# pain7576/ddpg-trucktrailer

Hardware: AMD Instinct MI355X
Metric: env-steps/s (higher is better)
Workload: dtype f64

## Files before the change

### ddpg-trucktrailer_amd/_lib.py

```python
import ctypes as C
import os

HERE = os.path.dirname(os.path.abspath(__file__))
LIB_PATH = os.environ.get("TT_LIB_PATH") or os.path.join(HERE, "libttenv.so")

OBS_DIM = 23
MAX_EPISODE_STEPS = 4095
TT_OK, TT_EINVAL, TT_ENOMEM, TT_EHIP, TT_ENODEV = 0, -1, -2, -3, -4
F_JACKKNIFE, F_OUT_OF_MAP, F_MAX_STEPS, F_GOAL_REACHED, F_GOAL_PASSED, F_EXCESSIVE_BACK, F_SUCCESS = (1 << i for i in range(7))
VIOLATIONS = ("none", "jackknife", "jackknife_warning", "major_boundary", "minor_boundary", "past_the_goal",
              "max_step", "excessive_backward")
INFO_ROWS = ("total_reward", "progress_reward", "heading_reward", "orientation_reward", "staged_success",
             "safety_penalty", "exploration_bonus", "final_success_bonus", "backward_penalty", "smoothness_penalty",
             "cumulative_backward", "movement_budget")
NINFO = len(INFO_ROWS)
LOG_COUNTS = ("episodes", "successes", "jackknife", "out_of_map", "max_steps", "goal_reached", "goal_passed",
              "excessive_back", "success_flag")
LOG_DETAIL = 1
LOG_COMPONENTS = INFO_ROWS[1:10]


class TTParams(C.Structure):
    _fields_ = [(n, C.c_double) for n in ("L1", "L2", "hitch_offset", "v1x", "dt", "map_min_x", "map_max_x", "map_min_y",
                                          "map_max_y", "max_steer", "position_threshold", "orientation_threshold",
                                          "step_length")] + \
               [("extra_steps", C.c_int32), ("fixed_max_steps", C.c_int32), ("term_mask", C.c_uint32),
                ("variant", C.c_int32), ("stateless_reward", C.c_int32), ("reserved_", C.c_int32),
                ("goal", C.c_double * 3), ("reset_lo", C.c_double * 3),
                ("reset_hi", C.c_double * 3)]


class TTInfo(C.Structure):
    _fields_ = [("comp", C.c_void_p), ("violation", C.c_void_p), ("flags", C.c_void_p)]


class TTMlpWeights(C.Structure):
    _fields_ = [(n, C.c_void_p) for n in ("w1", "b1", "g1", "be1", "w2", "b2", "g2", "be2", "w3", "b3", "wa", "ba")] + \
               [("in_dim", C.c_int32), ("fc1_dims", C.c_int32), ("fc2_dims", C.c_int32), ("capped_grids", C.c_int32),
                ("split_ws", C.c_void_p), ("ws_packed", C.c_int32), ("max_workgroups", C.c_int32), ("split_ws_alt", C.c_void_p), ("fc2_img", C.c_void_p)]


class TTFc2Images(C.Structure):
    _fields_ = [("net", C.c_void_p), ("target", C.c_void_p)]


class TTMlpSaved(C.Structure):
    _fields_ = [(n, C.c_void_p) for n in ("xh1", "h1", "xh2", "h2", "rstd1", "rstd2")]


class TTFwdJob(C.Structure):
    _fields_ = [("critic", C.c_int32), ("reserved_", C.c_int32), ("obs", C.c_void_p), ("action", C.c_void_p),
                ("w", C.POINTER(TTMlpWeights)), ("out", C.c_void_p), ("saved", C.POINTER(TTMlpSaved)),
                ("dq_da", C.c_void_p), ("z_state", C.c_void_p)]

# ... 145 lines not shown
    "tt_adam_soft_update": (C.c_int, [_I, _P, _P, _P, _P, _P, _P, _P, C.c_float, C.c_float, C.c_float, C.c_float,
                                      C.c_float, C.c_float, C.POINTER(TTFc2Images), _P, _P]),
    "tt_p2p_create": (C.c_int, [_I, _I, _I, _I, _P, C.POINTER(_P)]),
    "tt_p2p_destroy": (C.c_int, [_P]),
    "tt_p2p_export": (C.c_int, [_P, _P]),
    "tt_p2p_attach": (C.c_int, [_P, _I, _P]),
    "tt_p2p_grad": (_P, [_P, _I]),
    "tt_p2p_reset": (C.c_int, [_P, _P]),
    "tt_p2p_set_timeout": (C.c_int, [_P, C.c_double]),
    "tt_p2p_gave_up": (C.c_int, [_P]),
    "tt_p2p_last_error": (C.c_char_p, [_P]),
    "tt_adam_soft_update_p2p": (C.c_int, [_P, _I, _I, _P, _P, _P, _P, _P, _P, C.c_float, C.c_float, C.c_float, C.c_float,
                                          C.c_float, C.c_float, C.POINTER(TTFc2Images), _P, _P]),
    "tt_mlp_fc2_image_bytes": (C.c_uint64, []),
    "tt_mlp_fc2_image_pack": (C.c_int, [C.POINTER(TTMlpWeights), _P]),
    "tt_random_actions": (C.c_int, [_I, _U64, _U64, _P, _P]),
    "tt_pop_learn_create": (C.c_int, [_I, _I, C.POINTER(TTPopAgent), C.POINTER(_P)]),
    "tt_pop_learn": (C.c_int, [_P, _I, _P]),
    "tt_pop_learn_destroy": (C.c_int, [_P]),
    "tt_pop_exploit": (C.c_int, [_P, _I, C.POINTER(TTPopExploitPair), _P]),
    "tt_pop_hyper": (C.c_int, [_P, _I, C.POINTER(C.c_float * 4)]),
    "tt_pop_learn_set_nstep": (C.c_int, [_P, C.POINTER(TTPopNstep)]),
    "tt_pop_exploit_nstep": (C.c_int, [_P, _I, C.POINTER(TTPopExploitPair), C.POINTER(TTPopNstep), _P]),
    "tt_pop_nstep": (C.c_int, [_P, _I, C.POINTER(TTPopNstep)]),
    "tt_learn_log_create": (C.c_int, [_I, _I, C.POINTER(TTLearnLogJob), C.c_int64, C.c_int32, C.POINTER(_P)]),
    "tt_learn_log_append": (C.c_int, [_P, _P]),
    "tt_learn_log_drain": (C.c_int, [_P, _I, C.c_int64, C.c_int64, _P, _P, _P, C.POINTER(C.c_int64)]),
    "tt_learn_log_clear": (C.c_int, [_P, _P]),
    "tt_learn_log_destroy": (C.c_int, [_P]),
    "tt_td3_create": (C.c_int, [_I, C.POINTER(TTTd3Agent), C.POINTER(_P)]),
# ... 53 lines not shown
```

### ddpg-trucktrailer_amd/csrc/ttlearn.hip

```cpp
#include "ttlearn_bodies.h"
#include "ttp2p.h"

namespace {

template <bool CRITIC>
__global__ __launch_bounds__(64 * NW) void k_fwd_small(const int n, const float *__restrict__ obs,
                                                   const float *__restrict__ action, const float *__restrict__ w1e,
                                                   const float *__restrict__ b1e, const float *__restrict__ g1e,
                                                   const float *__restrict__ be1e, const Weights W,
                                                   float *__restrict__ out, const Saved sv, float *__restrict__ dq_da,
                                                   float *__restrict__ z_state) {
    __shared__ __attribute__((aligned(16))) float h1_s[H1S_FLOATS];
    __shared__ __attribute__((aligned(16))) float z_s[TR * DS];
    __shared__ __attribute__((aligned(16))) float w1_s[H1 * IN];
    KernargWarm<64 + (int)sizeof(Weights) + 8 + (int)sizeof(Saved) + 16> warm;
    warm.issue();
    KBEGIN(3);
    const EarlyW E{w1e, b1e, g1e, be1e};
    auto hook = [&]() __attribute__((always_inline)) { warm.wait(); };
    fwd_small_body<CRITIC, decltype(hook)>(n, obs, action, W, out, sv, dq_da, z_state, h1_s, z_s, w1_s, blockIdx.x * TR, nullptr, false, 0.f,
                                           0.f, nullptr, 0u, &E, hook);
    KEND(3);
}

__global__ __launch_bounds__(64 * NW) void k_fwd_multi(const FwdJobs J) {
    __shared__ __attribute__((aligned(16))) float h1_s[H1S_FLOATS];
    __shared__ __attribute__((aligned(16))) float z_s[TR * DS];
    __shared__ __attribute__((aligned(16))) float w1_s[H1 * IN];
    kernarg_warm<(int)sizeof(FwdJobs)>();
    const int job = blockIdx.x / J.blocks_per_job, row0 = (blockIdx.x - job * J.blocks_per_job) * TR;
    const FwdJob &q = J.j[job];
    KBEGIN(0);
#ifdef TT_STAMPS
    if (blockIdx.x == 0 && threadIdx.x < 64) {
        unsigned long long m = 0;
        for (int i = threadIdx.x; i < 512; i += 64) m = max(m, g_kblk[4][i][1]);
        for (int o = 32; o > 0; o >>= 1) m = max(m, (unsigned long long)__shfl_xor((long long)m, o));
        if (threadIdx.x == 0) g_kblk[5][0][0] = m;
    }
// ... 26 lines not shown
                        J.R.a_out[b] = ttnet::ring_pick_a(J.R, p);
                        if (J.R.idx_out) { J.R.idx_out[2 * b] = p.side ? -1 : p.t; J.R.idx_out[2 * b + 1] = p.side ? p.j : p.e; }
                    }
                }
                if (job == J.write_s2) {
                    J.R.s2_out[(size_t)b * ttnet::IN + c] = ttnet::ring_pick_s2(J.R, p)[c];
                    if (c == 0) { J.R.r_out[b] = ttnet::ring_pick_r(J.R, p); J.R.d_out[b] = ttnet::ring_pick_d(J.R, p); }
                }
            }
        }
    }
    if (q.critic)
        fwd_small_body<true>(J.n, q.obs, q.action, q.W, q.out, q.sv, q.dq_da, q.z_state, h1_s, z_s, w1_s, row0, orow, have_act, act_r0, act_r1);
    else
        fwd_small_body<false>(J.n, q.obs, q.action, q.W, q.out, q.sv, nullptr, nullptr, h1_s, z_s, w1_s, row0, orow);
    KEND(0);
}

__global__ __launch_bounds__(64 * NW) void k_bwd_rows_pair(const int n, const float scale_c, const float *__restrict__ q_out,
                                                           const Weights Wc, const Saved sv_c, const BwdOut o_c, const TdIn td,
                                                           const float *__restrict__ mu_out, const Weights Wa, const Saved sv_a,
                                                           const BwdOut o_a, const ImageJob img) {
    __shared__ __attribute__((aligned(16))) float dx2_s[DXS_FLOATS];
    __shared__ float red[2 * NW * TR];
    __shared__ float rsc_s[TR];
    kernarg_warm<16 + 2 * ((int)sizeof(Weights) + (int)sizeof(Saved) + (int)sizeof(BwdOut)) + (int)sizeof(TdIn) + 8>();
    const int nb = (n + TR - 1) / TR;
    if ((int)blockIdx.x == 2 * nb) {
        if (threadIdx.x == 0) clock_tick(td);
        return;
// ... 194 lines not shown
    const int nn = i / H1, k = i - nn * H1;
    img_store(img, nn, k, w2[i], true);
}

}

extern "C" {

int tt_mlp_forward_save(int n, int critic, const float *obs, const float *action, const tt_mlp_weights *w, float *out,
                        const tt_mlp_saved *saved, float *dq_da, tt_stream_t stream) {
    if (n < 0 || !obs || !out || !ok_shape(w, critic != 0) || (critic && !action)) return TT_EINVAL;
    if (n == 0) return TT_OK;
    Saved sv{nullptr, nullptr, nullptr, nullptr, nullptr, nullptr};
    if (saved && !to_saved(saved, sv)) return TT_EINVAL;
    const dim3 grid((n + TR - 1) / TR), block(64 * NW);
    if (critic)
        hipLaunchKernelGGL(k_fwd_small<true>, grid, block, 0, stream, n, obs, action, w->w1, w->b1, w->g1, w->be1, to_weights(w), out, sv, dq_da,
                           static_cast<float *>(nullptr));
    else
        hipLaunchKernelGGL(k_fwd_small<false>, grid, block, 0, stream, n, obs, action, w->w1, w->b1, w->g1, w->be1, to_weights(w), out, sv,
                           static_cast<float *>(nullptr), static_cast<float *>(nullptr));
    return hipGetLastError() == hipSuccess ? TT_OK : TT_EHIP;
}

static int forward_multi_impl(int n, int count, const tt_fwd_job *jobs, const tt_sample_args *sample, int64_t *k_snapshot,
                              tt_stream_t stream) {
    if (n < 0 || count < 1 || count > 4 || !jobs) return TT_EINVAL;
    if (n == 0) return TT_OK;
    FwdJobs J{};
    J.n = n;
    J.blocks_per_job = (n + TR - 1) / TR;
    J.write_s = J.write_s2 = -1;
    if (sample) {
        if (sample->batch != n) return TT_EINVAL;
        const int rc = ttnet::make_ring_sample(sample, J.R);
        if (rc != TT_OK) return rc;
        J.sampled = 1;
        J.R.progress = const_cast<int *>(sample->step_progress);
        J.k_snapshot = reinterpret_cast<long long *>(k_snapshot);
    }
    for (int i = 0; i < count; ++i)
        if (!to_fwd_job(jobs[i], i, sample, J)) return TT_EINVAL;
    if (sample && (J.write_s < 0 || J.write_s2 < 0)) return TT_EINVAL;
    hipLaunchKernelGGL(k_fwd_multi, dim3(count * J.blocks_per_job), dim3(64 * NW), 0, stream, J);
    return hipGetLastError() == hipSuccess ? TT_OK : TT_EHIP;
}

int tt_mlp_forward_multi(int n, int count, const tt_fwd_job *jobs, tt_stream_t stream) {
    return forward_multi_impl(n, count, jobs, nullptr, nullptr, stream);
}

int tt_mlp_forward_multi_sampled(int n, int count, const tt_fwd_job *jobs, const tt_sample_args *sample, int64_t *k_snapshot,
                                 tt_stream_t stream) {
    if (!sample) return TT_EINVAL;
    return forward_multi_impl(n, count, jobs, sample, k_snapshot, stream);
}

int tt_mlp_backward_rows_pair(int n, float scale_critic, const float *q_out, const tt_mlp_weights *critic,
                              const tt_mlp_saved *saved_critic, const tt_mlp_bwd_ws *ws_critic, const tt_td_input *tdi,
// ... 125 lines not shown
    X.world = x->world; X.me = x->rank; X.site = site;
    for (int r = 0; r < x->world; ++r) {
        if (!x->attached[r] || !x->block[r] || !x->flags[r]) return TT_EINVAL;
        X.arrive[r] = reinterpret_cast<int *>(x->flags[r]);
        X.grad[r] = reinterpret_cast<const float *>(x->block[r] + x->offset[site]);
    }
    X.gave_up_host = x->gave_up_host;
    X.wait_ticks = x->wait_ticks;
    hipLaunchKernelGGL(k_adam_soft_p2p, dim3(blocks), dim3(256), 0, stream, T, X, reinterpret_cast<const long long *>(step_dev), lr,
                       beta1, beta2, eps, weight_decay, tau, bias_corr);
    return hipGetLastError() == hipSuccess ? TT_OK : TT_EHIP;
}

uint64_t tt_mlp_fc2_image_bytes(void) { return (uint64_t)IMG_HALVES * 2; }

int tt_mlp_fc2_image_pack(const tt_mlp_weights *w, tt_stream_t stream) {
    if (!w || !w->w2 || !w->fc2_img || w->fc1_dims != H1 || w->fc2_dims != H2) return TT_EINVAL;
    hipLaunchKernelGGL(k_img_pack, dim3((H2 * H1 + 255) / 256), dim3(256), 0, stream, w->w2,
                       reinterpret_cast<_Float16 *>(w->fc2_img));
    return hipGetLastError() == hipSuccess ? TT_OK : TT_EHIP;
}

#ifdef TT_STAMPS
int tt_debug_blocks(unsigned long long *out1024) {
    return hipMemcpyFromSymbol(out1024, HIP_SYMBOL(g_blk), sizeof(unsigned long long) * 1024) == hipSuccess ? 0 : -3;
}
int tt_debug_wst(unsigned long long *out32) {
    return hipMemcpyFromSymbol(out32, HIP_SYMBOL(g_wst), sizeof(unsigned long long) * 32) == hipSuccess ? 0 : -3;
}
int tt_debug_kblocks(unsigned long long *out6x1024) {
// ... 21 lines not shown
```

### ddpg-trucktrailer_amd/csrc/ttlearn_bodies.h

```cpp
#pragma once
#include <hip/hip_runtime.h>

#include <cstdint>

#include "ttenv.h"
#include "ttnet_common.h"
#include "ttnet_pack.h"
#include "ttstamps.h"

namespace {

constexpr int IN = 23, INP = 24;
constexpr int H1 = 400, H2 = 300, H2P = 320, H2K = 304;
constexpr int NT1 = H1 / 16, NT2 = H2P / 16;
constexpr int TR = 16;
constexpr int NW = 8;
constexpr int HS1 = 404;

constexpr int DS = 308;

using f32x4 = __attribute__((ext_vector_type(4))) float;
using f16x8 = __attribute__((ext_vector_type(8))) _Float16;

constexpr int K2P = 416;
// ... 164 lines not shown
__device__ __forceinline__ float4 f4_ldu(const float *p) { return *reinterpret_cast<const float4 *>(p); }
__device__ __forceinline__ float f4_sum(const float4 v) { return (v.x + v.y) + (v.z + v.w); }
using h2v = __attribute__((ext_vector_type(2))) _Float16;
__device__ __forceinline__ void split4(const float4 x, uint2 &ph, uint2 &pm) {
    h2v a, b, c, d;
    a[0] = (_Float16)x.x; a[1] = (_Float16)x.y; b[0] = (_Float16)x.z; b[1] = (_Float16)x.w;
    c[0] = (_Float16)(x.x - (float)a[0]); c[1] = (_Float16)(x.y - (float)a[1]);
    d[0] = (_Float16)(x.z - (float)b[0]); d[1] = (_Float16)(x.w - (float)b[1]);
    ph = make_uint2(__builtin_bit_cast(uint32_t, a), __builtin_bit_cast(uint32_t, b));
    pm = make_uint2(__builtin_bit_cast(uint32_t, c), __builtin_bit_cast(uint32_t, d));
}

struct EarlyW {
    const float *__restrict__ w1, *__restrict__ b1, *__restrict__ g1, *__restrict__ be1;
};
template <bool CRITIC, class Hook = NoHook>
__device__ __forceinline__ void fwd_small_body(const int n, const float *__restrict__ obs,
                                               const float *__restrict__ action, const Weights &W,
                                               float *__restrict__ out, const Saved &sv, float *__restrict__ dq_da,
                                               float *__restrict__ z_state, float *__restrict__ h1_s,
                                               float *__restrict__ z_s, float *__restrict__ w1_s, const int row0,
                                               const float *__restrict__ obs_row_lane = nullptr,
                                               const bool act_given = false, const float act_row0 = 0.f,
                                               const float act_row1 = 0.f, unsigned long long *dq_words = nullptr,
                                               const unsigned dq_epoch = 0u, const EarlyW *early = nullptr,
                                               const Hook &loads_issued = Hook()) {
    const EarlyW E = early ? *early : EarlyW{W.w1, W.b1, W.g1, W.be1};
    const int tid = threadIdx.x, wave = tid >> 6, lane = tid & 63, l15 = lane & 15, l4 = lane >> 4;

    STAMP(0);
    constexpr int MT1 = (NT1 + NW - 1) / NW, MT2 = (NT2 + NW - 1) / NW;
    float4 pb1[RV], pg1[RV], pbe1[RV], pb2[RV], pg2[RV], pbe2[RV], pw3[RV], pwa[RV], pba[RV];
#pragma unroll
    for (int i = 0; i < RV; ++i) {
        const int c = rv_col(lane, i), cc = c < H1 ? c : 0;
        pb1[i] = *reinterpret_cast<const float4 *>(E.b1 + cc); pg1[i] = *reinterpret_cast<const float4 *>(E.g1 + cc);
        pbe1[i] = *reinterpret_cast<const float4 *>(E.be1 + cc);
    }
    f32x4 acc1[MT1];
#pragma unroll
    for (int i = 0; i < MT1; ++i) acc1[i] = f32x4{0.f, 0.f, 0.f, 0.f};
    constexpr int GU_F = 3;
    const bool img = W.img != nullptr;
    const int nt_f = (NT2 - wave + NW - 1) / NW;
    f16x8 bpre[GU_F][MT2][2];
    {
        float a[INP / 4];
        const float *arow = obs_row_lane ? obs_row_lane : obs + (size_t)min(row0 + l15, n - 1) * IN;
        const bool arow_ok = row0 + l15 < n;
        constexpr int W1_F4 = H1 * IN / 4, W1_PER = (W1_F4 + 64 * NW - 1) / (64 * NW);
        float4 wv[W1_PER];
#pragma unroll
        for (int q = 0; q < W1_PER; ++q) wv[q] = f4_ldu(E.w1 + 4 * min(tid + 64 * NW * q, W1_F4 - 1));
#pragma unroll
        for (int ks = 0; ks < INP / 4; ++ks) a[ks] = arow[min(ks * 4 + l4, IN - 1)];
        loads_issued();
        SUB(0);
#pragma unroll
        for (int q = 0; q < W1_PER; ++q)
            if (tid + 64 * NW * q < W1_F4) *reinterpret_cast<float4 *>(w1_s + 4 * (tid + 64 * NW * q)) = wv[q];
// ... 5 lines not shown
        float b[MT1][INP / 4];
#pragma unroll
        for (int i = 0; i < MT1; ++i) {
            const float *wr = w1_s + (min(wave + NW * i, NT1 - 1) * 16 + l15) * IN;
#pragma unroll
            for (int ks = 0; ks < INP / 4; ++ks) {
                const float v = wr[min(ks * 4 + l4, IN - 1)];
                b[i][ks] = ks * 4 + l4 < IN ? v : 0.f;
            }
        }
#pragma unroll
        for (int ks = 0; ks < INP / 4; ++ks)
#pragma unroll
            for (int i = 0; i < MT1; ++i)
                if (wave + NW * i < NT1) acc1[i] = __builtin_amdgcn_mfma_f32_16x16x4f32(a[ks], b[i][ks], acc1[i], 0, 0, 0);
        if (img) {
#pragma unroll
            for (int u = 0; u < GU_F; ++u)
#pragma unroll
                for (int i = 0; i < MT2; ++i) {
                    const _Float16 *bq = W.img + ((size_t)min(wave + NW * i, NT2 - 1) * FW_STEPS * 64 + lane) * 8 + 512 * u;
                    bpre[u][i][0] = *reinterpret_cast<const f16x8 *>(bq);
                    bpre[u][i][1] = *reinterpret_cast<const f16x8 *>(bq + IMG_FWD);
                }
        }
    }
    STAMP(1);
#pragma unroll
    for (int i = 0; i < MT1; ++i) {
        const int t = wave + NW * i;
        if (t < NT1) {
#pragma unroll
            for (int r = 0; r < 4; ++r) h1_s[(l4 * 4 + r) * HS1 + t * 16 + l15] = acc1[i][r];
        }
    }
    SUB(3);
    lds_barrier();
    SUB(4);
    _Float16 *const ap_s = reinterpret_cast<_Float16 *>(h1_s);
// ... 14 lines not shown
#pragma unroll
    for (int rr = 0; rr < TR / NW; ++rr) {
        const int lr = wave * (TR / NW) + rr, row = row0 + lr;
        const float mean = wave_sum64(f4_sum(xr[rr][0]) + f4_sum(xr[rr][1])) * (1.f / H1);
        float4 dv[RV];
        float ss = 0.f;
#pragma unroll
        for (int i = 0; i < RV; ++i) {
            const bool ok = rv_col(lane, i) < H1;
            const float4 x = xr[rr][i];
            dv[i] = ok ? make_float4(x.x - mean, x.y - mean, x.z - mean, x.w - mean) : f4_zero();
            ss = fmaf(dv[i].x, dv[i].x, ss); ss = fmaf(dv[i].y, dv[i].y, ss);
            ss = fmaf(dv[i].z, dv[i].z, ss); ss = fmaf(dv[i].w, dv[i].w, ss);
        }
        const float rstd = rsqrtf(wave_sum64(ss) * (1.f / H1) + 1e-5f);
        if (sv.rstd1 && lane == 0 && row < n) sv.rstd1[row] = rstd;
        const bool save = sv.xh1 && row < n;
#pragma unroll
        for (int i = 0; i < RV; ++i) {
            const int c = rv_col(lane, i);
            if (c < H1) {
                const float4 xh = make_float4(dv[i].x * rstd, dv[i].y * rstd, dv[i].z * rstd, dv[i].w * rstd);
                const float4 h = make_float4(fmaxf(fmaf(xh.x, pg1[i].x, pbe1[i].x), 0.f), fmaxf(fmaf(xh.y, pg1[i].y, pbe1[i].y), 0.f),
                                             fmaxf(fmaf(xh.z, pg1[i].z, pbe1[i].z), 0.f), fmaxf(fmaf(xh.w, pg1[i].w, pbe1[i].w), 0.f));
                if (img) {
                    uint2 ph, pm;
                    split4(make_float4(h.x * SXL, h.y * SXL, h.z * SXL, h.w * SXL), ph, pm);
                    *reinterpret_cast<uint2 *>(ap_s + lr * HSH + c) = ph;
                    *reinterpret_cast<uint2 *>(ap_s + TR * HSH + lr * HSH + c) = pm;
                } else {
                    *reinterpret_cast<float4 *>(&h1_s[lr * HS1 + c]) = h;
                }
// ... 20 lines not shown
            else { pwa[i] = f4_zero(); pba[i] = f4_zero(); }
        }
    };

    f32x4 acc2[MT2];
#pragma unroll
    for (int i = 0; i < MT2; ++i) acc2[i] = f32x4{0.f, 0.f, 0.f, 0.f};
    const float *wrow[MT2];
    bool wreal[MT2];
#pragma unroll
    for (int i = 0; i < MT2; ++i) {
        const int nn = (wave + NW * i) * 16 + l15;
        wreal[i] = wave + NW * i < NT2 && nn < H2;
        wrow[i] = W.w2 + (size_t)(wreal[i] ? nn : 0) * H1 + 4 * l4;
    }
    if (img) {
        const int nt = nt_f;
        const _Float16 *ah = ap_s + l15 * HSH + 8 * l4;
        const _Float16 *bh[MT2];
#pragma unroll
        for (int i = 0; i < MT2; ++i) bh[i] = W.img + ((size_t)min(wave + NW * i, NT2 - 1) * FW_STEPS * 64 + lane) * 8;
        constexpr int NS = FW_STEPS, GU = 3, NGRP = (NS + GU - 1) / GU;
        f16x8 bcur[GU][MT2][2], bnxt[GU][MT2][2];
        auto load_group = [&](const int g, f16x8 (&dst)[GU][MT2][2]) {
#pragma unroll
            for (int u = 0; u < GU; ++u)
#pragma unroll
                for (int i = 0; i < MT2; ++i) {
                    const int c = g * GU + u;
                    if (c < NS && i < nt) {
                        dst[u][i][0] = *reinterpret_cast<const f16x8 *>(bh[i] + 512 * c);
// ... 46 lines not shown
            bv[i] = *reinterpret_cast<const float4 *>(wrow[i] + 16 * c);
            if (!wreal[i]) bv[i] = make_float4(0.f, 0.f, 0.f, 0.f);
        }
#pragma unroll
        for (int i = 0; i < MT2; ++i) acc2[i] = __builtin_amdgcn_mfma_f32_16x16x4f32(av.x, bv[i].x, acc2[i], 0, 0, 0);
#pragma unroll
        for (int i = 0; i < MT2; ++i) acc2[i] = __builtin_amdgcn_mfma_f32_16x16x4f32(av.y, bv[i].y, acc2[i], 0, 0, 0);
#pragma unroll
        for (int i = 0; i < MT2; ++i) acc2[i] = __builtin_amdgcn_mfma_f32_16x16x4f32(av.z, bv[i].z, acc2[i], 0, 0, 0);
#pragma unroll
        for (int i = 0; i < MT2; ++i) acc2[i] = __builtin_amdgcn_mfma_f32_16x16x4f32(av.w, bv[i].w, acc2[i], 0, 0, 0);
    }
    }

    STAMP(3);
#pragma unroll
    for (int i = 0; i < MT2; ++i) {
        const int col = (wave + NW * i) * 16 + l15;
        if (wave + NW * i < NT2 && col < H2) {
#pragma unroll
            for (int r = 0; r < 4; ++r) z_s[(l4 * 4 + r) * DS + col] = acc2[i][r];
        }
    }
    lds_barrier();
    float avs[TR / NW];
#pragma unroll
    for (int rr = 0; rr < TR / NW; ++rr) {
        const int row = row0 + wave * (TR / NW) + rr;
        avs[rr] = (CRITIC && !z_state && row < n) ? (act_given ? (rr == 0 ? act_row0 : act_row1) : action[row]) : 0.f;
    }
    const float b3 = W.b3[0];
#pragma unroll
    for (int rr = 0; rr < TR / NW; ++rr) {
        const int lr = wave * (TR / NW) + rr, row = row0 + lr;
        float4 x[RV];
#pragma unroll
        for (int i = 0; i < RV; ++i) {
// ... 877 lines not shown
    int numel[MAXT], block_start[MAXT + 1];
    int count;
    _Float16 *img_p, *img_t;
};

Weights to_weights(const tt_mlp_weights *w) {
    return Weights{w->w1, w->b1, w->g1, w->be1, w->w2, w->b2, w->g2, w->be2, w->w3, w->b3, w->wa, w->ba,
                   reinterpret_cast<const _Float16 *>(w->fc2_img)};
}

bool ok_shape(const tt_mlp_weights *w, bool critic) {
    return w && w->in_dim == IN && w->fc1_dims == H1 && w->fc2_dims == H2 && w->w1 && w->b1 && w->g1 && w->be1 && w->w2 &&
           w->b2 && w->g2 && w->be2 && w->w3 && w->b3 && (!critic || (w->wa && w->ba));
}

bool to_saved(const tt_mlp_saved *s, Saved &sv) {
    if (!s || !s->xh1 || !s->h1 || !s->xh2 || !s->h2 || !s->rstd1 || !s->rstd2) return false;
    sv = Saved{s->xh1, s->h1, s->xh2, s->h2, s->rstd1, s->rstd2};
    return true;
}

bool to_bwd_out(const tt_mlp_bwd_ws *w, BwdOut &o) {
    if (!w || !w->dpre || !w->dz || !w->dx2 || !w->dy1 || !w->dx1) return false;
    o = BwdOut{w->dpre, w->dz, w->dx2, w->dy1, w->dx1};
    return true;
}

Grads to_grads(const tt_mlp_weights *g) {
    return Grads{const_cast<float *>(g->w1), const_cast<float *>(g->b1), const_cast<float *>(g->g1), const_cast<float *>(g->be1),
                 const_cast<float *>(g->w2), const_cast<float *>(g->b2), const_cast<float *>(g->g2), const_cast<float *>(g->be2),
// ... 49 lines not shown
```

### ddpg-trucktrailer_amd/fused_learn.py

```python
import ctypes as C

import torch

from ddpg_trucktrailer_amd import _lib as L
from ddpg_trucktrailer_amd import fused
from ddpg_trucktrailer_amd.replay_buffer import check_n_step

_p = L.ptr

_ORDER = ("fc1.weight", "fc1.bias", "bn1.weight", "bn1.bias", "fc2.weight", "fc2.bias", "bn2.weight", "bn2.bias")
_FIELDS = ("w1", "b1", "g1", "be1", "w2", "b2", "g2", "be2", "w3", "b3", "wa", "ba")


def _named(net):
    d = dict(net.named_parameters())
    head = "mu" if hasattr(net, "mu") else "q"
    names = list(_ORDER) + [head + ".weight", head + ".bias"]
    if hasattr(net, "action_value"):
        names += ["action_value.weight", "action_value.bias"]
    return [d[n] for n in names]


def _no_sync():
    return None
# ... 115 lines not shown
        cap, after = self.capacity, self.cursor[a]
        step, bad = np.empty(cap, np.int64), np.empty(cap, np.int32)
        vals = np.empty((len(L.LEARN_LOG_VALUES), cap), np.float64)
        n = C.c_int64(0)
        L.check(self.lib.tt_learn_log_drain(self._h, int(a), after, cap, step.ctypes.data, vals.ctypes.data, bad.ctypes.data, C.byref(n)))
        n = int(n.value)
        now = int(self.learners[a].step_dev.item())
        out = {"step": step[:n].copy(), "nonfinite": bad[:n].copy()}
        for name, col in zip(L.LEARN_LOG_VALUES, vals):
            out[name] = col[:n].copy()
        out["dropped"] = max(0, now // self.every - after // self.every) - n
        self.cursor[a] = max(now, after)
        return out


class FusedLearner:
    def __init__(self, agent, batch_size, fc2_images=None):
        import os
        assert fused.supported(agent.actor) and fused.supported(agent.critic)
        self.agent, self.B = agent, int(batch_size)
        dev = self.dev = agent.actor.fc1.weight.device
        self.lib = L.load()
        self.critic = _NetState(agent.critic, agent.target_critic, self.B, dev)
        self.actor = _NetState(agent.actor, agent.target_actor, self.B, dev)
        self.use_images = (os.environ.get("TT_LEARN_F32") != "1") if fc2_images is None else bool(fc2_images)
        self._wstruct, self._img, self._img_seen = {}, {}, {}
        for net in self._nets():
            self._make_weights(net)
        for st in (self.actor, self.critic):
            st.images = L.TTFc2Images(net=self._img_ptr(st.net), target=self._img_ptr(st.target)) if self.use_images else None
        f = dict(dtype=torch.float32, device=dev)
        B = self.B
        self.ws_t = dict(dpre=torch.empty(B, **f), dz=torch.empty((B, 300), **f), dx2=torch.empty((B, 300), **f),
                         dy1=torch.empty((B, 400), **f), dx1=torch.empty((B, 400), **f))
        self.ws = L.TTMlpBwdWs(**{k: v.data_ptr() for k, v in self.ws_t.items()})
        self.ws_actor_t = {k: torch.empty_like(v) for k, v in self.ws_t.items()}
        self.ws_actor = L.TTMlpBwdWs(**{k: v.data_ptr() for k, v in self.ws_actor_t.items()})
        self.mu_t, self.q_t, self.y, self.q, self.mu, self.q_pi, self.dq_da = (torch.empty(B, **f) for _ in range(7))
        self.step_dev = torch.zeros((), dtype=torch.int64, device=dev)
        self.bias_corr = torch.zeros(8, dtype=torch.float32, device=dev)
# ... 9 lines not shown
        self.hyp_critic = (gc["lr"], gc["betas"][0], gc["betas"][1], gc["eps"], gc["weight_decay"])

    def _nets(self):
        ag = self.agent
        return (ag.actor, ag.critic, ag.target_actor, ag.target_critic)

    def _states(self):
        return (self.actor, self.critic)

    def _make_weights(self, net):
        w = fused._fill_weights(net, L.TTMlpWeights())
        if self.use_images:
            img = torch.zeros(int(self.lib.tt_mlp_fc2_image_bytes()), dtype=torch.uint8, device=self.dev)
            self._img[id(net)] = img
            w.fc2_img = img.data_ptr()
        self._wstruct[id(net)] = (tuple(p.data_ptr() for p in net.parameters()), w)
        self._img_seen[id(net)] = None

    def _img_ptr(self, net):
        t = self._img.get(id(net))
        return None if t is None else t.data_ptr()

    def w(self, net):
        key, w = self._wstruct[id(net)]
        if key != tuple(p.data_ptr() for p in net.parameters()):
            self._make_weights(net)
            for st in self._states():
                if self.use_images:
                    st.images = L.TTFc2Images(net=self._img_ptr(st.net), target=self._img_ptr(st.target))
            w = self._wstruct[id(net)][1]
# ... 136 lines not shown
                L.check(self.lib.tt_mlp_forward_multi_sampled(B, 4, jobs, C.byref(sample), snap, self._stream()))
        else:
            L.check(self.lib.tt_mlp_forward_multi(B, 4, jobs, self._stream()))
        self._rows(rewards, done_u8, window_dev, image, n_step)
        self._weights(self.critic, self.hyp_critic, ag.tau, states, actions, self.ws, adam=fuse_adam)

    def fwd_jobs(self, states, actions, states_):
        ag = self.agent
        jobs = (L.TTFwdJob * 4)()
        for j, (net, crit, obs, act, out, saved, zst) in enumerate((
                (ag.target_actor, 0, states_, None, self.mu_t, None, None),
                (ag.target_critic, 1, states_, None, None, None, self.z_t),
                (ag.critic, 1, states, actions, self.q, self.critic.saved, None),
                (ag.actor, 0, states, None, self.mu, self.actor.saved, None))):
            jobs[j].critic, jobs[j].obs, jobs[j].action = crit, L.ptr(obs), L.ptr(act)
            jobs[j].w, jobs[j].out = C.pointer(self.w(net)), L.ptr(out)
            jobs[j].saved = C.pointer(saved) if saved is not None else None
            jobs[j].dq_da, jobs[j].z_state = None, L.ptr(zst)
        return jobs

    def td_input(self, rewards, done_u8, window_dev=None, n_step=1):
        ag = self.agent
        gamma = nstep_discount(ag.gamma, n_step)
        return L.TTTdInput(z_state=self.z_t.data_ptr(), mu_target=self.mu_t.data_ptr(),
                           target_critic=C.pointer(self.w(ag.target_critic)), reward=rewards.data_ptr(),
                           done=done_u8.data_ptr(), gamma=gamma, y_out=self.y.data_ptr(),
                           q_out=self.q_t.data_ptr(), step_dev=self.step_dev.data_ptr(), window_dev=L.ptr(window_dev),
                           bias_corr_out=self.bias_corr.data_ptr(), adam_beta1=self.hyp_critic[1], adam_beta2=self.hyp_critic[2])

    def _rows(self, rewards, done_u8, window_dev=None, image=None, n_step=1):
        ag, B = self.agent, self.B
# ... 85 lines not shown
```

### include/ttenv.h

```cpp
#ifndef TTENV_H
#define TTENV_H

#include <stddef.h>
#include <stdint.h>

#ifdef __cplusplus
extern "C" {
#endif

#define TT_VERSION 3
#define TT_OBS_DIM 23
#define TT_MAX_EPISODE_STEPS 4095

enum { TT_OK = 0, TT_EINVAL = -1, TT_ENOMEM = -2, TT_EHIP = -3, TT_ENODEV = -4 };

enum {
    TT_F_JACKKNIFE = 1, TT_F_OUT_OF_MAP = 2, TT_F_MAX_STEPS = 4, TT_F_GOAL_REACHED = 8,
    TT_F_GOAL_PASSED = 16, TT_F_EXCESSIVE_BACK = 32, TT_F_SUCCESS = 64
};
#define TT_TERM_SIMV2 0x3F
#define TT_TERM_SIMV1 0x0F

enum {
    TT_V_NONE = 0, TT_V_JACKKNIFE, TT_V_JACKKNIFE_WARNING, TT_V_MAJOR_BOUNDARY, TT_V_MINOR_BOUNDARY,
// ... 113 lines not shown

int tt_env_profile(tt_env *env, int max_launches);
int tt_env_profile_read(tt_env *env, double *total_ms, int64_t *launches);

int tt_random_actions(int n, uint64_t seed, uint64_t step, float *out, tt_stream_t stream);

typedef struct tt_mlp_weights {
    const float *w1, *b1, *g1, *be1, *w2, *b2, *g2, *be2, *w3, *b3, *wa, *ba;
    int32_t in_dim, fc1_dims, fc2_dims;
    int32_t capped_grids;
    void *split_ws;
    int32_t ws_packed;
    int32_t max_workgroups;
    void *split_ws_alt;
    void *fc2_img;
} tt_mlp_weights;
uint64_t tt_mlp_fc2_image_bytes(void);
int tt_mlp_fc2_image_pack(const tt_mlp_weights *w, tt_stream_t stream);
typedef struct tt_fc2_images {
    void *net, *target;
} tt_fc2_images;
uint64_t tt_mlp_split_ws_bytes(void);
int tt_mlp_split_pack(const tt_mlp_weights *w, int critic, void *ws, int64_t *bump, const tt_ring_cursor *cursor,
                      tt_stream_t stream);

int tt_actor_forward(int n, const float *obs , const tt_mlp_weights *w, float *mu_out, tt_stream_t stream);

int tt_actor_act(int n, const float *obs, const tt_mlp_weights *w, float *ou_state, const uint8_t *done_prev,
                 uint64_t seed, uint64_t step, const int64_t *step_dev, float theta_dt, float sigma_sqrt_dt, float high,
                 float *mu_out, float *act_raw_out, float *act_scaled_out, tt_stream_t stream);

// ... 206 lines not shown
```

Measured before the change: 807.0 million.

## Split fc2 forward tiles across multiple workgroups with atomic last-block reduction

Adds a column-split mode where each row group's fc2 forward GEMM is divided across 2 or 4 workgroups. Each one computes a slice of the output tiles from the packed fp16 image and writes its partial z to a global workspace. The last-arriving block, found through an atomic counter, gathers z into LDS and finishes the layer. This is meant to raise parallelism and occupancy for small batches, and it defaults to 4 slices for the plain FusedLearner. The cost is an extra global round-trip, an atomic handshake per group, and redundant fc1 work in every slice.

```diff
diff --git a/ddpg-trucktrailer_amd/_lib.py b/ddpg-trucktrailer_amd/_lib.py
--- a/ddpg-trucktrailer_amd/_lib.py
+++ b/ddpg-trucktrailer_amd/_lib.py
@@ -37,7 +37,8 @@
 class TTMlpWeights(C.Structure):
     _fields_ = [(n, C.c_void_p) for n in ("w1", "b1", "g1", "be1", "w2", "b2", "g2", "be2", "w3", "b3", "wa", "ba")] + \
                [("in_dim", C.c_int32), ("fc1_dims", C.c_int32), ("fc2_dims", C.c_int32), ("capped_grids", C.c_int32),
-                ("split_ws", C.c_void_p), ("ws_packed", C.c_int32), ("max_workgroups", C.c_int32), ("split_ws_alt", C.c_void_p), ("fc2_img", C.c_void_p)]
+                ("split_ws", C.c_void_p), ("ws_packed", C.c_int32), ("max_workgroups", C.c_int32), ("split_ws_alt", C.c_void_p), ("fc2_img", C.c_void_p),
+                ("colsplit_ws", C.c_void_p), ("colsplit", C.c_int32), ("reserved2_", C.c_int32)]
 
 
 class TTFc2Images(C.Structure):
@@ -213,6 +214,9 @@
                                           C.c_float, C.c_float, C.POINTER(TTFc2Images), _P, _P]),
     "tt_mlp_fc2_image_bytes": (C.c_uint64, []),
     "tt_mlp_fc2_image_pack": (C.c_int, [C.POINTER(TTMlpWeights), _P]),
+    "tt_mlp_colsplit_ws_bytes": (C.c_uint64, [_I]),
+    "tt_mlp_colsplit_check": (C.c_int, [_I]),
+    "tt_mlp_colsplit_slice": (C.c_int, [_I, _I, _I, _P, _P]),
     "tt_random_actions": (C.c_int, [_I, _U64, _U64, _P, _P]),
     "tt_pop_learn_create": (C.c_int, [_I, _I, C.POINTER(TTPopAgent), C.POINTER(_P)]),
     "tt_pop_learn": (C.c_int, [_P, _I, _P]),
diff --git a/ddpg-trucktrailer_amd/csrc/ttlearn.hip b/ddpg-trucktrailer_amd/csrc/ttlearn.hip
--- a/ddpg-trucktrailer_amd/csrc/ttlearn.hip
+++ b/ddpg-trucktrailer_amd/csrc/ttlearn.hip
@@ -23,6 +23,28 @@
     KEND(3);
 }
 
+template <bool CRITIC, int COLS>
+__global__ __launch_bounds__(64 * NW) void k_fwd_small_cols(const int n, const float *__restrict__ obs,
+                                                        const float *__restrict__ action, const float *__restrict__ w1e,
+                                                        const float *__restrict__ b1e, const float *__restrict__ g1e,
+                                                        const float *__restrict__ be1e, const Weights W,
+                                                        float *__restrict__ out, const Saved sv, float *__restrict__ dq_da,
+                                                        float *__restrict__ z_state, float *__restrict__ cs_z, unsigned *cs_count) {
+    __shared__ __attribute__((aligned(16))) float h1_s[H1S_FLOATS];
+    __shared__ __attribute__((aligned(16))) float z_s[TR * DS];
+    __shared__ __attribute__((aligned(16))) float w1_s[H1 * IN];
+    KernargWarm<64 + (int)sizeof(Weights) + 8 + (int)sizeof(Saved) + 16 + 16> warm;
+    warm.issue();
+    KBEGIN(3);
+    const EarlyW E{w1e, b1e, g1e, be1e};
+    auto hook = [&]() __attribute__((always_inline)) { warm.wait(); };
+    const int group = blockIdx.x / COLS;
+    const ColSlice cs{cs_z + (size_t)group * (TR * H2), cs_count + group, (int)blockIdx.x - group * COLS};
+    fwd_small_body<CRITIC, decltype(hook), COLS>(n, obs, action, W, out, sv, dq_da, z_state, h1_s, z_s, w1_s, group * TR, nullptr, false, 0.f,
+                                                 0.f, nullptr, 0u, &E, hook, cs);
+    KEND(3);
+}
+
 __global__ __launch_bounds__(64 * NW) void k_fwd_multi(const FwdJobs J) {
     __shared__ __attribute__((aligned(16))) float h1_s[H1S_FLOATS];
     __shared__ __attribute__((aligned(16))) float z_s[TR * DS];
@@ -79,6 +101,73 @@
         fwd_small_body<true>(J.n, q.obs, q.action, q.W, q.out, q.sv, q.dq_da, q.z_state, h1_s, z_s, w1_s, row0, orow, have_act, act_r0, act_r1);
     else
         fwd_small_body<false>(J.n, q.obs, q.action, q.W, q.out, q.sv, nullptr, nullptr, h1_s, z_s, w1_s, row0, orow);
+    KEND(0);
+}
+
+struct ColJobs {
+    float *z[4];
+    unsigned *count[4];
+};
+template <int COLS>
+__global__ __launch_bounds__(64 * NW) void k_fwd_multi_cols(const FwdJobs J, const ColJobs CJ) {
+    __shared__ __attribute__((aligned(16))) float h1_s[H1S_FLOATS];
+    __shared__ __attribute__((aligned(16))) float z_s[TR * DS];
+    __shared__ __attribute__((aligned(16))) float w1_s[H1 * IN];
+    kernarg_warm<(int)sizeof(FwdJobs) + (int)sizeof(ColJobs)>();
+    const int per_job = J.blocks_per_job * COLS, job = blockIdx.x / per_job, rem = (int)blockIdx.x - job * per_job;
+    const int group = rem / COLS, slice = rem - group * COLS, row0 = group * TR;
+    const FwdJob &q = J.j[job];
+    const ColSlice cs{CJ.z[job] + (size_t)group * (TR * H2), CJ.count[job] + group, slice};
+    KBEGIN(0);
+#ifdef TT_STAMPS
+    if (blockIdx.x == 0 && threadIdx.x < 64) {
+        unsigned long long m = 0;
+        for (int i = threadIdx.x; i < 512; i += 64) m = max(m, g_kblk[4][i][1]);
+        for (int o = 32; o > 0; o >>= 1) m = max(m, (unsigned long long)__shfl_xor((long long)m, o));
+        if (threadIdx.x == 0) g_kblk[5][0][0] = m;
+    }
+#endif
+    const float *orow = nullptr;
+    bool have_act = false;
+    float act_r0 = 0.f, act_r1 = 0.f;
+    if (J.sampled) {
+        ttnet::await_progress(J.R.progress, J.R.k_dev);
+        const int tid = threadIdx.x, wave = tid >> 6, l15 = tid & 15;
+        if (J.k_snapshot && blockIdx.x == 0 && tid == 0) *J.k_snapshot = *J.R.k_dev;
+        const bool from_s = q.obs == J.R.s_out;
+        {
+            const ttnet::RingPick p = ttnet::ring_sample_index(J.R, min(row0 + l15, J.n - 1));
+            orow = from_s ? ttnet::ring_pick_s(J.R, p) : ttnet::ring_pick_s2(J.R, p);
+        }
+        if (q.critic && q.action) {
+            act_r0 = ttnet::ring_pick_a(J.R, ttnet::ring_sample_index(J.R, min(row0 + wave * 2, J.n - 1)));
+            act_r1 = ttnet::ring_pick_a(J.R, ttnet::ring_sample_index(J.R, min(row0 + wave * 2 + 1, J.n - 1)));
+            have_act = true;
+        }
+        if (slice == 0 && (job == J.write_s || job == J.write_s2)) {
+            const int lr = tid / ttnet::IN, c = tid - lr * ttnet::IN, b = row0 + lr;
+            if (lr < TR && b < J.n) {
+                const ttnet::RingPick p = ttnet::ring_sample_index(J.R, b);
+                if (job == J.write_s) {
+                    J.R.s_out[(size_t)b * ttnet::IN + c] = ttnet::ring_pick_s(J.R, p)[c];
+                    if (c == 0) {
+                        J.R.a_out[b] = ttnet::ring_pick_a(J.R, p);
+                        if (J.R.idx_out) { J.R.idx_out[2 * b] = p.side ? -1 : p.t; J.R.idx_out[2 * b + 1] = p.side ? p.j : p.e; }
+                    }
+                }
+                if (job == J.write_s2) {
+                    J.R.s2_out[(size_t)b * ttnet::IN + c] = ttnet::ring_pick_s2(J.R, p)[c];
+                    if (c == 0) { J.R.r_out[b] = ttnet::ring_pick_r(J.R, p); J.R.d_out[b] = ttnet::ring_pick_d(J.R, p); }
+                }
+            }
+        }
+    }
+    if (q.critic)
+        fwd_small_body<true, NoHook, COLS>(J.n, q.obs, q.action, q.W, q.out, q.sv, q.dq_da, q.z_state, h1_s, z_s, w1_s, row0, orow, have_act,
+                                           act_r0, act_r1, nullptr, 0u, nullptr, NoHook(), cs);
+    else
+        fwd_small_body<false, NoHook, COLS>(J.n, q.obs, q.action, q.W, q.out, q.sv, nullptr, nullptr, h1_s, z_s, w1_s, row0, orow, false, 0.f,
+                                            0.f, nullptr, 0u, nullptr, NoHook(), cs);
     KEND(0);
 }
 
@@ -303,6 +392,20 @@
     Saved sv{nullptr, nullptr, nullptr, nullptr, nullptr, nullptr};
     if (saved && !to_saved(saved, sv)) return TT_EINVAL;
     const dim3 grid((n + TR - 1) / TR), block(64 * NW);
+    const int cols = colsplit_of(w);
+    if (cols < 0) return TT_EINVAL;
+    if (cols > 1) {
+        const ColWs cw = colsplit_ws(w, n);
+        const dim3 gridc(grid.x * cols);
+        float *const none = nullptr;
+#define TT_FWD_COLS(CR, C_)                                                                                                        \
+    hipLaunchKernelGGL((k_fwd_small_cols<CR, C_>), gridc, block, 0, stream, n, obs, action, w->w1, w->b1, w->g1, w->be1, to_weights(w), \
+                       out, sv, CR ? dq_da : none, none, cw.z, cw.count)
+        if (critic) { if (cols == 2) TT_FWD_COLS(true, 2); else TT_FWD_COLS(true, 4); }
+        else { if (cols == 2) TT_FWD_COLS(false, 2); else TT_FWD_COLS(false, 4); }
+#undef TT_FWD_COLS
+        return hipGetLastError() == hipSuccess ? TT_OK : TT_EHIP;
+    }
     if (critic)
         hipLaunchKernelGGL(k_fwd_small<true>, grid, block, 0, stream, n, obs, action, w->w1, w->b1, w->g1, w->be1, to_weights(w), out, sv, dq_da,
                            static_cast<float *>(nullptr));
@@ -331,7 +434,20 @@
     for (int i = 0; i < count; ++i)
         if (!to_fwd_job(jobs[i], i, sample, J)) return TT_EINVAL;
     if (sample && (J.write_s < 0 || J.write_s2 < 0)) return TT_EINVAL;
-    hipLaunchKernelGGL(k_fwd_multi, dim3(count * J.blocks_per_job), dim3(64 * NW), 0, stream, J);
+    int cols = colsplit_of(jobs[0].w);
+    ColJobs CJ{};
+    for (int i = 0; i < count; ++i) {
+        if (cols < 0 || colsplit_of(jobs[i].w) != cols) return TT_EINVAL;
+        if (cols > 1) {
+            const ColWs cw = colsplit_ws(jobs[i].w, n);
+            for (int k = 0; k < i; ++k)
+                if (CJ.z[k] == cw.z) return TT_EINVAL;
+            CJ.z[i] = cw.z; CJ.count[i] = cw.count;
+        }
+    }
+    if (cols == 2) hipLaunchKernelGGL(k_fwd_multi_cols<2>, dim3(count * J.blocks_per_job * 2), dim3(64 * NW), 0, stream, J, CJ);
+    else if (cols == 4) hipLaunchKernelGGL(k_fwd_multi_cols<4>, dim3(count * J.blocks_per_job * 4), dim3(64 * NW), 0, stream, J, CJ);
+    else hipLaunchKernelGGL(k_fwd_multi, dim3(count * J.blocks_per_job), dim3(64 * NW), 0, stream, J);
     return hipGetLastError() == hipSuccess ? TT_OK : TT_EHIP;
 }
 
@@ -487,6 +603,18 @@
 
 uint64_t tt_mlp_fc2_image_bytes(void) { return (uint64_t)IMG_HALVES * 2; }
 
+uint64_t tt_mlp_colsplit_ws_bytes(int n) { return n > 0 ? (uint64_t)colsplit_ws_bytes(n) : 0; }
+
+int tt_mlp_colsplit_check(int cols) { return colsplit_ok(cols) ? TT_OK : TT_EINVAL; }
+
+int tt_mlp_colsplit_slice(int cols, int slice, int backward, int32_t *first_tile, int32_t *tiles) {
+    if (!colsplit_ok(cols) || slice < 0 || slice >= (cols < 1 ? 1 : cols) || !first_tile || !tiles) return TT_EINVAL;
+    const int c = cols < 1 ? 1 : cols, per = (backward ? BW_TILES : FW_TILES) / c;
+    *first_tile = slice * per;
+    *tiles = per;
+    return TT_OK;
+}
+
 int tt_mlp_fc2_image_pack(const tt_mlp_weights *w, tt_stream_t stream) {
     if (!w || !w->w2 || !w->fc2_img || w->fc1_dims != H1 || w->fc2_dims != H2) return TT_EINVAL;
     hipLaunchKernelGGL(k_img_pack, dim3((H2 * H1 + 255) / 256), dim3(256), 0, stream, w->w2,
diff --git a/ddpg-trucktrailer_amd/csrc/ttlearn_bodies.h b/ddpg-trucktrailer_amd/csrc/ttlearn_bodies.h
--- a/ddpg-trucktrailer_amd/csrc/ttlearn_bodies.h
+++ b/ddpg-trucktrailer_amd/csrc/ttlearn_bodies.h
@@ -202,7 +202,12 @@
 struct EarlyW {
     const float *__restrict__ w1, *__restrict__ b1, *__restrict__ g1, *__restrict__ be1;
 };
-template <bool CRITIC, class Hook = NoHook>
+struct ColSlice {
+    float *__restrict__ z;
+    unsigned *count;
+    int slice;
+};
+template <bool CRITIC, class Hook = NoHook, int COLS = 1>
 __device__ __forceinline__ void fwd_small_body(const int n, const float *__restrict__ obs,
                                                const float *__restrict__ action, const Weights &W,
                                                float *__restrict__ out, const Saved &sv, float *__restrict__ dq_da,
@@ -212,7 +217,11 @@
                                                const bool act_given = false, const float act_row0 = 0.f,
                                                const float act_row1 = 0.f, unsigned long long *dq_words = nullptr,
                                                const unsigned dq_epoch = 0u, const EarlyW *early = nullptr,
-                                               const Hook &loads_issued = Hook()) {
+                                               const Hook &loads_issued = Hook(), const ColSlice cs = ColSlice{nullptr, nullptr, 0}) {
+    static_assert(COLS >= 1 && FW_TILES % COLS == 0, "the slices cover the 20 forward tiles exactly once");
+    constexpr int TPS = FW_TILES / COLS;
+    constexpr int TW = (TPS + NW - 1) / NW;
+    static_assert(COLS == 1 || TW <= 3, "a wave's tiles fit acc2");
     const EarlyW E = early ? *early : EarlyW{W.w1, W.b1, W.g1, W.be1};
     const int tid = threadIdx.x, wave = tid >> 6, lane = tid & 63, l15 = lane & 15, l4 = lane >> 4;
 
@@ -232,6 +241,17 @@
     const bool img = W.img != nullptr;
     const int nt_f = (NT2 - wave + NW - 1) / NW;
     f16x8 bpre[GU_F][MT2][2];
+    f16x8 bsl[COLS > 1 ? FW_STEPS : 1][2];
+    auto load_slice_tile = [&](const int t) __attribute__((always_inline)) {
+        if constexpr (COLS > 1) {
+            const _Float16 *bq = W.img + ((size_t)(cs.slice * TPS + t) * FW_STEPS * 64 + lane) * 8;
+#pragma unroll
+            for (int c = 0; c < FW_STEPS; ++c) {
+                bsl[c][0] = *reinterpret_cast<const f16x8 *>(bq + 512 * c);
+                bsl[c][1] = *reinterpret_cast<const f16x8 *>(bq + IMG_FWD + 512 * c);
+            }
+        }
+    };
     {
         float a[INP / 4];
         const float *arow = obs_row_lane ? obs_row_lane : obs + (size_t)min(row0 + l15, n - 1) * IN;
@@ -267,7 +287,7 @@
 #pragma unroll
             for (int i = 0; i < MT1; ++i)
                 if (wave + NW * i < NT1) acc1[i] = __builtin_amdgcn_mfma_f32_16x16x4f32(a[ks], b[i][ks], acc1[i], 0, 0, 0);
-        if (img) {
+        if (COLS == 1 && img) {
 #pragma unroll
             for (int u = 0; u < GU_F; ++u)
 #pragma unroll
@@ -276,6 +296,9 @@
                     bpre[u][i][0] = *reinterpret_cast<const f16x8 *>(bq);
                     bpre[u][i][1] = *reinterpret_cast<const f16x8 *>(bq + IMG_FWD);
                 }
+        }
+        if constexpr (COLS > 1) {
+            if (wave < TPS) load_slice_tile(wave);
         }
     }
     STAMP(1);
@@ -320,8 +343,9 @@
             ss = fmaf(dv[i].z, dv[i].z, ss); ss = fmaf(dv[i].w, dv[i].w, ss);
         }
         const float rstd = rsqrtf(wave_sum64(ss) * (1.f / H1) + 1e-5f);
-        if (sv.rstd1 && lane == 0 && row < n) sv.rstd1[row] = rstd;
-        const bool save = sv.xh1 && row < n;
+        const bool saver = COLS == 1 || cs.slice == 0;
+        if (sv.rstd1 && lane == 0 && row < n && saver) sv.rstd1[row] = rstd;
+        const bool save = sv.xh1 && row < n && saver;
 #pragma unroll
         for (int i = 0; i < RV; ++i) {
             const int c = rv_col(lane, i);
@@ -372,7 +396,25 @@
         wreal[i] = wave + NW * i < NT2 && nn < H2;
         wrow[i] = W.w2 + (size_t)(wreal[i] ? nn : 0) * H1 + 4 * l4;
     }
-    if (img) {
+    if constexpr (COLS > 1) {
+        load_l2_vectors();
+#pragma unroll
+        for (int tw = 0; tw < TW; ++tw) {
+            if (wave + NW * tw < TPS) {
+                if (tw > 0) load_slice_tile(wave + NW * tw);
+                const _Float16 *ah = ap_s + l15 * HSH + 8 * l4;
+#pragma unroll
+                for (int c = 0; c < FW_STEPS; ++c) {
+                    const f16x8 a_h = *reinterpret_cast<const f16x8 *>(ah + 32 * c);
+                    const f16x8 a_m = *reinterpret_cast<const f16x8 *>(ah + TR * HSH + 32 * c);
+                    acc2[tw] = mfma_h(a_m, bsl[c][0], acc2[tw]);
+                    acc2[tw] = mfma_h(a_h, bsl[c][1], acc2[tw]);
+                    acc2[tw] = mfma_h(a_h, bsl[c][0], acc2[tw]);
+                }
+                acc2[tw] *= UNSC_L;
+            }
+        }
+    } else if (img) {
         const int nt = nt_f;
         const _Float16 *ah = ap_s + l15 * HSH + 8 * l4;
         const _Float16 *bh[MT2];
@@ -449,6 +491,45 @@
     }
 
     STAMP(3);
+    if constexpr (COLS > 1) {
+#pragma unroll
+        for (int tw = 0; tw < TW; ++tw) {
+            const int col = (cs.slice * TPS + wave + NW * tw) * 16 + l15;
+            if (wave + NW * tw < TPS && col < H2) {
+#pragma unroll
+                for (int r = 0; r < 4; ++r) cs.z[(l4 * 4 + r) * H2 + col] = acc2[tw][r];
+            }
+        }
+        int *const last_s = reinterpret_cast<int *>(w1_s);
+        asm volatile("s_waitcnt vmcnt(0)" ::: "memory");
+        __syncthreads();
+        if (tid == 0) {
+            __builtin_amdgcn_fence(__ATOMIC_RELEASE, "agent");
+            asm volatile("s_waitcnt vmcnt(0)" ::: "memory");
+            const unsigned before = __hip_atomic_fetch_add(cs.count, 1u, __ATOMIC_RELAXED, __HIP_MEMORY_SCOPE_AGENT);
+            const bool last = before == (unsigned)(COLS - 1);
+            if (last) __hip_atomic_store(cs.count, 0u, __ATOMIC_RELAXED, __HIP_MEMORY_SCOPE_AGENT);
+            last_s[0] = last ? 1 : 0;
+        }
+        __syncthreads();
+        if (last_s[0] == 0) return;
+        SUB(7);
+        constexpr int ZW = TR * H2 / 2, ZPER = (ZW + 64 * NW - 1) / (64 * NW);
+        unsigned long long zw[ZPER];
+        const unsigned long long *zsrc = reinterpret_cast<const unsigned long long *>(cs.z);
+#pragma unroll
+        for (int q = 0; q < ZPER; ++q)
+            zw[q] = __hip_atomic_load(zsrc + min(tid + 64 * NW * q, ZW - 1), __ATOMIC_RELAXED, __HIP_MEMORY_SCOPE_AGENT);
+#pragma unroll
+        for (int q = 0; q < ZPER; ++q) {
+            const int e = tid + 64 * NW * q;
+            if (e < ZW) {
+                const int zr = e / (H2 / 2), zc = e - zr * (H2 / 2);
+                *reinterpret_cast<unsigned long long *>(&z_s[zr * DS + 2 * zc]) = zw[q];
+            }
+        }
+        SUB(8);
+    } else {
 #pragma unroll
     for (int i = 0; i < MT2; ++i) {
         const int col = (wave + NW * i) * 16 + l15;
@@ -456,6 +537,7 @@
 #pragma unroll
             for (int r = 0; r < 4; ++r) z_s[(l4 * 4 + r) * DS + col] = acc2[i][r];
         }
+    }
     }
     lds_barrier();
     float avs[TR / NW];
@@ -1363,6 +1445,23 @@
            w->b2 && w->g2 && w->be2 && w->w3 && w->b3 && (!critic || (w->wa && w->ba));
 }
 
+bool colsplit_ok(const int cols) { return cols == 0 || (cols > 0 && FW_TILES % cols == 0 && BW_TILES % cols == 0); }
+int colsplit_of(const tt_mlp_weights *w) {
+    if (!colsplit_ok(w->colsplit)) return -1;
+    if (w->colsplit <= 1 || !w->fc2_img) return 1;
+    return w->colsplit_ws ? w->colsplit : -1;
+}
+size_t colsplit_ws_counters(const int n) { return (((size_t)((n + TR - 1) / TR) * sizeof(unsigned)) + 255) / 256 * 256; }
+size_t colsplit_ws_bytes(const int n) { return colsplit_ws_counters(n) + (size_t)((n + TR - 1) / TR) * TR * H2 * sizeof(float); }
+struct ColWs {
+    float *z;
+    unsigned *count;
+};
+ColWs colsplit_ws(const tt_mlp_weights *w, const int n) {
+    unsigned char *p = static_cast<unsigned char *>(w->colsplit_ws);
+    return ColWs{reinterpret_cast<float *>(p + colsplit_ws_counters(n)), reinterpret_cast<unsigned *>(p)};
+}
+
 bool to_saved(const tt_mlp_saved *s, Saved &sv) {
     if (!s || !s->xh1 || !s->h1 || !s->xh2 || !s->h2 || !s->rstd1 || !s->rstd2) return false;
     sv = Saved{s->xh1, s->h1, s->xh2, s->h2, s->rstd1, s->rstd2};
diff --git a/ddpg-trucktrailer_amd/fused_learn.py b/ddpg-trucktrailer_amd/fused_learn.py
--- a/ddpg-trucktrailer_amd/fused_learn.py
+++ b/ddpg-trucktrailer_amd/fused_learn.py
@@ -153,8 +153,23 @@
         return out
 
 
+def learn_colsplit_default(lone=True):
+    import os
+    v = os.environ.get("TT_LEARN_COLSPLIT")
+    if v is not None and v.strip() != "":
+        return int(v)
+    return 4 if lone else 1
+
+
+def check_colsplit(cols):
+    cols = int(cols)
+    if cols < 1 or L.load().tt_mlp_colsplit_check(cols) != L.TT_OK:
+        raise ValueError(f"colsplit = {cols} does not divide the 20 forward and 28 backward tiles of the fc2 image (1, 2 or 4)")
+    return cols
+
+
 class FusedLearner:
-    def __init__(self, agent, batch_size, fc2_images=None):
+    def __init__(self, agent, batch_size, fc2_images=None, colsplit=None):
         import os
         assert fused.supported(agent.actor) and fused.supported(agent.critic)
         self.agent, self.B = agent, int(batch_size)
@@ -163,6 +178,10 @@
         self.critic = _NetState(agent.critic, agent.target_critic, self.B, dev)
         self.actor = _NetState(agent.actor, agent.target_actor, self.B, dev)
         self.use_images = (os.environ.get("TT_LEARN_F32") != "1") if fc2_images is None else bool(fc2_images)
+        self.colsplit = check_colsplit(learn_colsplit_default(type(self) is FusedLearner) if colsplit is None else colsplit)
+        cm = os.environ.get("TT_LEARN_COLSPLIT_MULTI")
+        self.colsplit_multi = check_colsplit(cm) if cm else self.colsplit
+        self._colsplit_ws, self._wmulti = {}, {}
         self._wstruct, self._img, self._img_seen = {}, {}, {}
         for net in self._nets():
             self._make_weights(net)
@@ -202,6 +221,16 @@
             img = torch.zeros(int(self.lib.tt_mlp_fc2_image_bytes()), dtype=torch.uint8, device=self.dev)
             self._img[id(net)] = img
             w.fc2_img = img.data_ptr()
+            if max(self.colsplit, self.colsplit_multi) > 1:
+                ws = self._colsplit_ws.get(id(net))
+                if ws is None:
+                    ws = torch.zeros(int(self.lib.tt_mlp_colsplit_ws_bytes(self.B)), dtype=torch.uint8, device=self.dev)
+                    self._colsplit_ws[id(net)] = ws
+                w.colsplit_ws, w.colsplit = ws.data_ptr(), self.colsplit
+        wm = L.TTMlpWeights()
+        C.memmove(C.byref(wm), C.byref(w), C.sizeof(w))
+        wm.colsplit = self.colsplit_multi if (self.use_images and wm.colsplit_ws) else 0
+        self._wmulti[id(net)] = wm
         self._wstruct[id(net)] = (tuple(p.data_ptr() for p in net.parameters()), w)
         self._img_seen[id(net)] = None
 
@@ -368,7 +397,8 @@
                 (ag.critic, 1, states, actions, self.q, self.critic.saved, None),
                 (ag.actor, 0, states, None, self.mu, self.actor.saved, None))):
             jobs[j].critic, jobs[j].obs, jobs[j].action = crit, L.ptr(obs), L.ptr(act)
-            jobs[j].w, jobs[j].out = C.pointer(self.w(net)), L.ptr(out)
+            self.w(net)
+            jobs[j].w, jobs[j].out = C.pointer(self._wmulti[id(net)]), L.ptr(out)
             jobs[j].saved = C.pointer(saved) if saved is not None else None
             jobs[j].dq_da, jobs[j].z_state = None, L.ptr(zst)
         return jobs
diff --git a/include/ttenv.h b/include/ttenv.h
--- a/include/ttenv.h
+++ b/include/ttenv.h
@@ -151,7 +151,13 @@
     int32_t max_workgroups;
     void *split_ws_alt;
     void *fc2_img;
+    void *colsplit_ws;
+    int32_t colsplit;
+    int32_t reserved2_;
 } tt_mlp_weights;
+uint64_t tt_mlp_colsplit_ws_bytes(int n);
+int tt_mlp_colsplit_check(int cols);
+int tt_mlp_colsplit_slice(int cols, int slice, int backward, int32_t *first_tile, int32_t *tiles);
 uint64_t tt_mlp_fc2_image_bytes(void);
 int tt_mlp_fc2_image_pack(const tt_mlp_weights *w, tt_stream_t stream);
 typedef struct tt_fc2_images {
```

Measured after the change: 734.5 million. 0.91x the previous value.
